# MorphIQ-Labs/VectorWave

Measured on AMD Instinct MI355X. Metric: Msamples/sec MODWT fwd+inv db4 L=6, batch 4096×4096 fp64 @ 1/2/4/8 GPU, higher is better.
Workload: dtype f64

## Files before the change

### vectorwave_amd/csrc/vw_device.h

```cpp
#pragma once
#include <hip/hip_runtime.h>
#include <cstdint>
#include <type_traits>
#include "vw_internal.h"

#pragma clang fp contract(off)

namespace vw {

template <typename T> struct VT;
template <> struct VT<double> { typedef double v __attribute__((ext_vector_type(2))); static constexpr int V = 2; };
template <> struct VT<float>  { typedef float  v __attribute__((ext_vector_type(4))); static constexpr int V = 4; };

__device__ __forceinline__ double fma_t(double a, double b, double c) { return __builtin_fma(a, b, c); }
__device__ __forceinline__ float fma_t(float a, float b, float c) { return __builtin_fmaf(a, b, c); }

template <bool FMA, typename T>
__device__ __forceinline__ T madd(T acc, T x, T f) {
  if constexpr (FMA) return fma_t(x, f, acc);
  else return acc + x * f;
}

#ifndef VW_PK_F32
#define VW_PK_F32 0
// ... 920 lines not shown
  const size_t plane = (size_t)p.B * (size_t)N;

  T reg[NV][V];
  T dnext[NV][V];
  load_row_regs<T, NV>(reg, p.approx + b * (size_t)N, N, nvec, vec_ok, p.approx_zero != 0);
  load_row_regs<T, NV>(dnext, p.details + (size_t)(p.J - 1) * plane + b * (size_t)N, N, nvec, vec_ok,
                       p.lv[p.J - 1].use_d == 0);
  wait_vmem();
  regs_to_level<T, L, NV>(A, reg, nvec, N, p.lv[p.J - 1], 0, (const T*)nullptr, p.approx_zero != 0);
  regs_to_level<T, L, NV>(D, dnext, nvec, N, p.lv[p.J - 1], 0, (const T*)nullptr, p.lv[p.J - 1].use_d == 0, p.thr,
                          thr_of(p.J), p.soft);

  for (int j = p.J; j >= 1; --j) {
    const LevelDesc lv = p.lv[j - 1];
    lds_barrier();
    if (j > 1) {
      load_row_regs<T, NV>(dnext, p.details + (size_t)(j - 2) * plane + b * (size_t)N, N, nvec, vec_ok,
                           p.lv[j - 2].use_d == 0);
    }
    for_vecs<L, NV>(nvec, [&](int k, int w) {
      T acc[V];
#pragma unroll
      for (int e = 0; e < V; ++e) acc[e] = T(0);
      inv_pair<T, L, FMA>(A, D, w * V, lv.s, lv.dir_a, p.lo, p.hi, p.taps, acc);
#pragma unroll
      for (int e = 0; e < V; ++e) {
        asm volatile("" : "+v"(acc[e]));
        reg[k][e] = acc[e];
      }
    });
    if (j == 1) {
      for_vecs<L, NV>(nvec, [&](int k, int w) { store_vec<VW_INV_STORE_AUX>(p.y + b * (size_t)N, w * V, N, vec_ok, reg[k]); });
    } else {
      const LevelDesc ln = p.lv[j - 2];
      lds_barrier();
      regs_to_level<T, L, NV>(A, reg, nvec, N, ln, 0, (const T*)nullptr);
      wait_vmem();
      regs_to_level<T, L, NV>(D, dnext, nvec, N, ln, 0, (const T*)nullptr, ln.use_d == 0, p.thr, thr_of(j - 1), p.soft);
    }
  }
}

template <typename T, int L, bool FMA, int NV, int LH = L>
__global__ void VW_FUSED_BOUNDS(NV, VW_FUSED_W((L > LH ? L : LH), 6)) k_inverse_db(const InvArgs<T> p) {
  constexpr int V = VT<T>::V;
  extern __shared__ __attribute__((aligned(16))) unsigned char smem[];
  T* const X = reinterpret_cast<T*>(smem) + p.hlpad_a;
  T* const Y = reinterpret_cast<T*>(smem) + p.region_d + p.hlpad_d;
  const long long b = p.rev ? p.B - 1 - (long long)blockIdx.x : (long long)blockIdx.x;
  const int N = p.N;
  const int nvec = (N + V - 1) / V;
  const bool vec_ok = (L > 0) || p.vec_io != 0;
  auto thr_of = [&](int j) { return p.thr ? load_uniform(p.thr + (size_t)(j - 1) * (size_t)p.thr_ld + (size_t)b) : T(0); };
  const size_t plane = (size_t)p.B * (size_t)N;

  T acc[NV][V];
  T dreg[NV][V];
  load_row_regs<T, NV>(acc, p.approx + b * (size_t)N, N, nvec, vec_ok, p.approx_zero != 0);
  load_row_regs<T, NV>(dreg, p.details + (size_t)(p.J - 1) * plane + b * (size_t)N, N, nvec, vec_ok,
                       p.lv[p.J - 1].use_d == 0);
  wait_vmem();
  regs_to_level<T, L, NV>(X, acc, nvec, N, p.lv[p.J - 1], 0, (const T*)nullptr, p.approx_zero != 0);

  for (int j = p.J; j >= 1; --j) {
    const LevelDesc lv = p.lv[j - 1];
    lds_barrier();
    wait_vmem();
    regs_to_level<T, L, NV>(Y, dreg, nvec, N, lv, 0, (const T*)nullptr, lv.use_d == 0, p.thr, thr_of(j), p.soft);
    if (j > 1)
      load_row_regs<T, NV>(dreg, p.details + (size_t)(j - 2) * plane + b * (size_t)N, N, nvec, vec_ok,
                           p.lv[j - 2].use_d == 0);
    zero_regs<T, NV>(acc);
    inv_row<T, L, FMA, NV>(X, nvec, lv.s, lv.dir_a, lv.off_a, p.lo, p.taps, p.level_ct, acc);
    lds_barrier();
    inv_row<T, LH, FMA, NV>(Y, nvec, lv.s, lv.dir_d, lv.off_d, p.hi, p.taps_hi, p.level_ct, acc);
    if (j > 1) regs_to_level<T, L, NV>(X, acc, nvec, N, p.lv[j - 2], 0, (const T*)nullptr);
  }
  for_vecs<L, NV>(nvec, [&](int k, int w) { store_vec<VW_INV_STORE_AUX>(p.y + b * (size_t)N, w * V, N, vec_ok, acc[k]); });
}

#ifndef VW_INV_W
#define VW_INV_W 6
#endif
template <typename T, int L, bool FMA, int NV, bool FULL = false, int LH = L>
__global__ void VW_FUSED_BOUNDS(NV, VW_FUSED_W((L > LH ? L : LH), VW_INV_W)) k_inverse_seq(const InvArgs<T> p) {
  constexpr int V = VT<T>::V;
  extern __shared__ __attribute__((aligned(16))) unsigned char smem[];
  T* R = reinterpret_cast<T*>(smem) + p.hlpad_a;
  const long long b = p.rev ? p.B - 1 - (long long)blockIdx.x : (long long)blockIdx.x;
  const int N = p.N;
  const int nvec = (N + V - 1) / V;
  const bool vec_ok = (L > 0) || p.vec_io != 0;
  auto thr_of = [&](int j) { return p.thr ? load_uniform(p.thr + (size_t)(j - 1) * (size_t)p.thr_ld + (size_t)b) : T(0); };
  const size_t plane = (size_t)p.B * (size_t)N;

  T acc[NV][V];
  T dreg[NV][V];
  T nf = T(0);
  const bool nfp = p.nf_flag != nullptr;
  load_row_regs<T, NV, FULL>(acc, p.approx + b * (size_t)N, N, nvec, vec_ok, p.approx_zero != 0);
  load_row_regs<T, NV, FULL>(dreg, p.details + (size_t)(p.J - 1) * plane + b * (size_t)N, N, nvec, vec_ok,
                       p.lv[p.J - 1].use_d == 0);
  wait_vmem();
  regs_to_level<T, L, NV, FULL>(R, acc, nvec, N, p.lv[p.J - 1], 0, (const T*)nullptr, p.approx_zero != 0);

  for (int j = p.J; j >= 1; --j) {
    const LevelDesc lv = p.lv[j - 1];
    lds_barrier();
    zero_regs<T, NV>(acc);
    inv_row<T, L, FMA, NV, FULL>(R, nvec, lv.s, lv.dir_a, lv.off_a, p.lo, p.taps, p.level_ct, acc);
    lds_barrier();
    wait_vmem();
    regs_to_level<T, L, NV, FULL>(R, dreg, nvec, N, lv, 0, (const T*)nullptr, lv.use_d == 0, p.thr, thr_of(j), p.soft);
    if (j > 1)
      load_row_regs<T, NV, FULL>(dreg, p.details + (size_t)(j - 2) * plane + b * (size_t)N, N, nvec, vec_ok,
                           p.lv[j - 2].use_d == 0);
    lds_barrier();
    inv_row<T, LH, FMA, NV, FULL>(R, nvec, lv.s, lv.dir_d, lv.off_d, p.hi, p.taps_hi, p.level_ct, acc);
    if (j > 1) {
      lds_barrier();
      regs_to_level<T, L, NV, FULL>(R, acc, nvec, N, p.lv[j - 2], 0, (const T*)nullptr);
    }
  }
  for_vecs<L, NV, FULL>(nvec, [&](int k, int w) { store_vec<VW_INV_STORE_AUX, FULL>(p.y + b * (size_t)N, w * V, N, vec_ok, acc[k]); });
  if (nfp) {
    nf_probe_rows<T, L, NV, V, FULL>(nf, acc, nvec);
    nf_flag_row<T>(p.nf_flag, b, nf);
  }
}

}

#include "vw_blk.h"

namespace vw {

template <typename T>
__device__ __forceinline__ T halo_value_global(const T* __restrict__ src, int idx, int N, int mode, int npow2,
                                               const T* hist_b, int hist_len) {
  if (idx >= 0 && idx < N) return src[idx];
  switch (mode) {
    case kHaloPeriodic: { int r = idx % N; if (r < 0) r += N; return src[r]; }
    case kHaloSymmetric: return src[sym_index(idx, N)];
    case kHaloFftPad: { int r = idx < 0 ? idx + npow2 : idx; return (r >= 0 && r < N) ? src[r] : T(0); }
    case kHaloHistory: return (idx < 0 && idx >= -hist_len) ? hist_b[hist_len + idx] : T(0);
    default: return T(0);
  }
}

template <typename T>
__device__ __forceinline__ void tile_to_lds(T* buf, const T* __restrict__ src, int N, int ts, int lo_q, int hi_q,
                                            int mode, int npow2, const T* hist_b, int hist_len, const T* thr,
                                            T thr_b, int soft, bool zero, bool vec_ok = false) {
  constexpr int V = VT<T>::V;
  using vec = typename VT<T>::v;
  int qa = lo_q, qb = lo_q;
  if (vec_ok && !zero) {
    qa = max(lo_q, -ts);
    qa = (qa + V - 1) / V * V;
    qb = min(hi_q, N - ts);
    qb = qb >= qa ? qa + (qb - qa) / V * V : qa;
  }
  for (int q = qa + (int)threadIdx.x * V; q < qb; q += blockDim.x * V) {
    vec v = __builtin_nontemporal_load(reinterpret_cast<const vec*>(src + ts + q));
    if (thr) {
#pragma unroll
      for (int e = 0; e < V; ++e) v[e] = threshold_t(v[e], thr_b, soft);
    }
// ... 767 lines not shown
```

### vectorwave_amd/csrc/vw_internal.h

```cpp
#pragma once
#include <hip/hip_runtime.h>
#include <atomic>
#include <cstdint>
#include "vw_taps.h"

namespace vw {

constexpr int kMaxTaps = 64;
constexpr int kMaxLevels = 24;
constexpr int kNV = 8;
constexpr int kMaxThreads = 1024;
constexpr int kLdsBytes = 160 * 1024;
constexpr int kSweepMinS = 16;
constexpr int kSweepChunk = 128;

enum HaloMode : int {
  kHaloPeriodic = 0,
  kHaloZero = 1,
  kHaloSymmetric = 2,
  kHaloFftPad = 3,
  kHaloHistory = 4
};

struct LevelDesc {
  int s;
  int hl, hr;
  int mode;
  int dir_a;
  int off_a;
  int dir_d;
  int off_d;
  int use_d;
  int hist_len;
  int own;
  int il_a, il_b;
  int ir_a, ir_b;
  int vs, ve;
};

template <typename T>
struct FwdArgs {
  const T* x;
  long long ldx;
  T* details;
  T* approx;
  long long B;
  int N;
  int J;
  int npow2;
  int hlpad;
  int region1;
  int vec_io;
  int unrolled;
  int dma_nt;
  int level_ct;
  int validate;
  int rev;
  unsigned long long* bad;
  T* hist[kMaxLevels];
  int hist_update;
  int taps;
  int taps_hi;
  int tap_lds;
  int blk_tight;
  int* nf_flag;
  T lo[kMaxTaps];
  T hi[kMaxTaps];
  LevelDesc lv[kMaxLevels];
};

template <typename T>
struct InvArgs {
  const T* details;
  const T* approx;
  T* y;
  long long B;
  int N;
  int J;
  int hlpad_a, hlpad_d;
  int region_d;
  int vec_io;
  int pair;
  int unrolled;
  int level_ct;
  int full;
  int db;
  int blk;
  int approx_zero;
  int rev;
  const T* thr;
  long long thr_ld;
  int soft;
  int taps;
  int taps_hi;
  int tap_lds;
  int blk_tight;
  int* nf_flag;
  T lo[kMaxTaps];
  T hi[kMaxTaps];
  LevelDesc lv[kMaxLevels];
};

template <typename T>
struct LevelArgs {
  const T* src_a;
  long long lda;
  const T* src_d;
  const T* src_d2;
  const T* thr2;
  int use_d2;
  const T* src_d3;
  const T* thr3;
  int use_d3;
  T* out_a;
  T* out_d;
  const T* hist;
  long long B;
  int N;
  int tile;
  int hlpad;
  int region_d, hlpad_d;
  int pair;
  const T* thr;
  int soft;
  int use_d;
  int vec_io;
  int validate;
  unsigned long long* bad;
  int npow2;
  int taps;
  T lo[kMaxTaps];
  T hi[kMaxTaps];
  LevelDesc lv;
};

constexpr int kMaxGroup = 8;
constexpr int kMultiInvNI = 8;
constexpr int kMultiPF = 6;
template <typename T>
struct MultiArgs {
  const T* src_a;
  long long lda;
  const T* src_d[kMaxGroup];
  T* out_d[kMaxGroup];
  T* out_a;
  const T* thr[kMaxGroup];
  long long B;
  int N;
  int tile;
  int nlev;
  int s0;
  int ext[kMaxGroup + 1];
  int region;
  int vec_io;
  int soft;
  int taps;
  int rblk;
  int pf;
  int pad;
  int* nf_flag;
  int slack;
  int ni;
  T lo[kMaxTaps];
  T hi[kMaxTaps];
};

enum ThrMethod { kThrUniversal = 0, kThrSure = 1, kThrMinimax = 2, kThrBayes = 3, kThrFixed = 4 };
constexpr int kSigmaRegN = 16384;
// ... 194 lines not shown
```

### vectorwave_amd/csrc/vw_inv.hip

```cpp
#include "vw_launch.h"
#include <algorithm>

namespace vw {

template <typename T, int L, bool FMA, int NV>
static hipError_t run_inverse_fused_nv(const InvArgs<T>& a, int threads, int lds, hipStream_t st) {
  static LdsOnce configured_pair, configured_seq, configured_db, configured_blk, configured_full;
  const bool blk = L > 0 && NV != 2 && a.blk && !a.pair && !a.db;
  auto k = a.pair ? k_inverse_fused<T, L, FMA, NV> : a.db ? k_inverse_db<T, L, FMA, NV> : k_inverse_seq<T, L, FMA, NV>;
  if constexpr (NV != 2) {
    if (blk) k = k_inverse_blk<T, (L > 0 ? L : 2), FMA, NV>;
  }
  bool full = false;
  if constexpr (NV == 4 && L > 0 && L <= 8) {
    full = a.full && !a.pair && !a.db && !blk;
    if (full) k = k_inverse_seq<T, L, FMA, NV, true>;
  }
  hipError_t e = set_lds(k, lds, a.pair ? &configured_pair : a.db ? &configured_db
                                 : blk ? &configured_blk : full ? &configured_full : &configured_seq);
  if (e != hipSuccess) return e;
  hipLaunchKernelGGL(k, dim3((unsigned)a.B), dim3(threads), lds, st, a);
  return hipGetLastError();
}

template <typename T, int L, bool FMA>
static hipError_t run_inverse_fused(const InvArgs<T>& a, int threads, int lds, int nv, hipStream_t st) {
  if constexpr (L > 0 && L <= 8) {
    if (nv == 2) return run_inverse_fused_nv<T, L, FMA, 2>(a, threads, lds, st);
  }
  return nv <= 4 ? run_inverse_fused_nv<T, L, FMA, 4>(a, threads, lds, st) : run_inverse_fused_nv<T, L, FMA, 8>(a, threads, lds, st);
}

template <typename T, int L, int LH, bool FMA, int NV>
static hipError_t run_inverse_bi_nv(const InvArgs<T>& a, int threads, int lds, hipStream_t st) {
  static LdsOnce configured_seq, configured_db;
  auto k = a.db ? k_inverse_db<T, L, FMA, NV, LH> : k_inverse_seq<T, L, FMA, NV, false, LH>;
  hipError_t e = set_lds(k, lds, a.db ? &configured_db : &configured_seq);
  if (e != hipSuccess) return e;
  hipLaunchKernelGGL(k, dim3((unsigned)a.B), dim3(threads), lds, st, a);
  return hipGetLastError();
}
template <typename T, int L, int LH>
static hipError_t run_inverse_bi(const InvArgs<T>& a, int threads, int lds, bool fma, int nv, hipStream_t st) {
  if (nv <= 4) return fma ? run_inverse_bi_nv<T, L, LH, true, 4>(a, threads, lds, st) : run_inverse_bi_nv<T, L, LH, false, 4>(a, threads, lds, st);
  return fma ? run_inverse_bi_nv<T, L, LH, true, 8>(a, threads, lds, st) : run_inverse_bi_nv<T, L, LH, false, 8>(a, threads, lds, st);
}

template <typename T>
hipError_t launch_inverse_fused(const InvArgs<T>& a, int threads, int lds, bool fma, int nv, hipStream_t st) {
  if (a.taps_hi != a.taps) {
    if (a.pair || a.blk || nv == 2) return hipErrorInvalidValue;
    if (a.unrolled) {
#define VW_CASE(lo, hi) if (a.taps == lo && a.taps_hi == hi) return run_inverse_bi<T, lo, hi>(a, threads, lds, fma, nv, st);
      VW_TAP_PAIR_LIST(VW_CASE)
#undef VW_CASE
    }
    return run_inverse_bi<T, 0, 0>(a, threads, lds, fma, nv, st);
  }
  switch (a.unrolled ? a.taps : 0) {
#define VW_CASE(n) \
    case n: return fma ? run_inverse_fused<T, n, true>(a, threads, lds, nv, st) : run_inverse_fused<T, n, false>(a, threads, lds, nv, st);
    VW_TAP_LIST(VW_CASE)
#undef VW_CASE
    default:
      return fma ? run_inverse_fused<T, 0, true>(a, threads, lds, nv, st) : run_inverse_fused<T, 0, false>(a, threads, lds, nv, st);
  }
}
template hipError_t launch_inverse_fused<VW_T>(const InvArgs<VW_T>&, int, int, bool, int, hipStream_t);
}
```

### vectorwave_amd/csrc/vw_plan.cpp

```cpp
#include "vw_plan.h"

#include <algorithm>
#include <cstdio>
#include <cstdlib>
#include <cstring>
#include <type_traits>

namespace vw {

struct TuningKey {
  const char* name;
  void (*set)(Tuning& t, const Tuning& d, int v);
};
#define VW_KEY(name, stmt) {name, [](Tuning& t, const Tuning& d, int v) { (void)d; stmt; }}
static const TuningKey kTuningTable[] = {
    VW_KEY("VW_NV", t.nv = v < 0 ? d.nv : v <= 4 ? 4 : 8),
    VW_KEY("VW_FWD_PERSIST", t.fwd_persist = v < 0 ? d.fwd_persist : v != 0),
    VW_KEY("VW_FWD_BUF", t.fwd_buf = v < 0 ? d.fwd_buf : v),
    VW_KEY("VW_FORCE_TILED", t.force_tiled = v > 0),
    VW_KEY("VW_FWD_REV", t.fwd_rev = v < 0 ? 0 : v),
    VW_KEY("VW_INV_REV", t.inv_rev = v < 0 ? 0 : v),
    VW_KEY("VW_FWD_TILE", t.fwd_tile = v < 0 ? 0 : v),
    VW_KEY("VW_MULTI", t.multi = v < 0 ? d.multi : v != 0),
    VW_KEY("VW_MULTI_DIV", t.multi_div = v <= 0 ? d.multi_div : v),
    VW_KEY("VW_MULTI_TILE", t.multi_tile = v < 0 ? 0 : v),
    VW_KEY("VW_INV_BUF", t.inv_buf = v < 0 ? 0 : v),
    VW_KEY("VW_INV_TILE", t.inv_tile = v < 0 ? 0 : v),
    VW_KEY("VW_MULTI_RBLK", t.multi_rblk = v < 0 ? d.multi_rblk : v),
    VW_KEY("VW_MULTI_PF", t.multi_pf = v < 0 ? d.multi_pf : v),
    VW_KEY("VW_MULTI_PAD", t.multi_pad = v < 0 ? d.multi_pad : v),
    VW_KEY("VW_MULTI_INV_TILE", t.multi_inv_tile = v < 0 ? 0 : v),
    VW_KEY("VW_NO_SWEEP", t.no_sweep = v > 0),
    VW_KEY("VW_SWEEP_QC", t.sweep_qc = v >= 16 ? v : d.sweep_qc),
    VW_KEY("VW_UNROLL_MAX", t.unroll_max = v < 0 ? d.unroll_max : v),
    VW_KEY("VW_BLK", t.blk = v < 0 ? d.blk : v),
    VW_KEY("VW_FWD_NV", t.fwd_nv = v < 0 ? d.fwd_nv : v),
    VW_KEY("VW_INV_NV", t.inv_nv = v < 0 ? d.inv_nv : v),
    VW_KEY("VW_DEEP", t.deep = v < 0 ? d.deep : v != 0; t.deep_inv = v < 0 ? d.deep_inv : v != 0),
    VW_KEY("VW_DEEP_INV", t.deep_inv = v < 0 ? d.deep_inv : v != 0),
    VW_KEY("VW_DEEP_LDS", t.deep_lds = v <= 0 ? d.deep_lds : v),
    VW_KEY("VW_DEEP_WAVES", t.deep_waves = v <= 0 ? d.deep_waves : v),
    VW_KEY("VW_DEEP_PF_FWD", t.deep_pf_fwd = v <= 0 ? d.deep_pf_fwd : std::min(v, 16)),
    VW_KEY("VW_DEEP_PF_INV", t.deep_pf_inv = v <= 0 ? d.deep_pf_inv : std::min(v, 16)),
    VW_KEY("VW_SWEEP2", t.sweep2 = v < 0 ? d.sweep2 : v),
    VW_KEY("VW_SWEEP2_KA", t.sweep2_ka = v == 16 ? 16 : v == 8 ? 8 : d.sweep2_ka),
    VW_KEY("VW_SWEEP2_UC", t.sweep2_uc = v >= 32 ? v : d.sweep2_uc),
    VW_KEY("VW_SWEEP2_R", t.sweep2_r = v == 32 ? 32 : 0),
    VW_KEY("VW_SWEEP2_MINB", t.sweep2_minb = v < 0 ? d.sweep2_minb : v),
    VW_KEY("VW_BLK_FWD8", t.blk_fwd8 = v < 0 ? d.blk_fwd8 : v),
    VW_KEY("VW_DMA_NT", t.dma_nt = v < 0 ? d.dma_nt : v),
    VW_KEY("VW_MULTI_NI", t.multi_ni = v < 0 ? d.multi_ni : v == 4 ? 4 : 8),
    VW_KEY("VW_MFMA", t.mfma = v < 0 ? d.mfma : v),
    VW_KEY("VW_REF_GRID", t.ref_grid = v < 0 ? d.ref_grid : v),
    VW_KEY("VW_LEVEL_CT", t.level_ct = v < 0 ? d.level_ct : v != 0),
    VW_KEY("VW_ENERGY_FUSED", t.energy_fused = v < 0 ? d.energy_fused : v),
    VW_KEY("VW_BI", t.bi = v < 0 ? d.bi : v & 7),
    VW_KEY("VW_BI_LISTED", t.bi_listed = v < 0 ? d.bi_listed : v != 0),
};
#undef VW_KEY

bool set_tuning(Tuning& t, const char* key, int v) {
  const Tuning d;
  for (const TuningKey& k : kTuningTable)
    if (!strcmp(k.name, key)) { k.set(t, d, v); return true; }
  return false;
}

Tuning read_tuning() {
  Tuning t;
  const Tuning d;
  for (const TuningKey& k : kTuningTable) {
    const char* e = getenv(k.name);
    if (e) k.set(t, d, *e == '\0' ? 1 : atoi(e));
  }
  return t;
}


int max_levels(int64_t N, int L) {
  if (L <= 0 || N <= L) return 0;
  int max_level = 1;
  const long long lm1 = L - 1;
  while (max_level < 10) {
    const long long scaled = lm1 * (1LL << (max_level - 1)) + 1LL;
    if (scaled > N) break;
    max_level++;
  }
  return max_level - 1;
}

int64_t upsampled_length(int L, int level) {
  const int64_t up = (level <= 1) ? 1 : ((int64_t)1 << (level - 1));
  return (int64_t)(L - 1) * up + 1;
}

int ref_mode(int boundary) {
  return boundary == VW_PERIODIC ? kHaloPeriodic : boundary == VW_ZERO_PADDING ? kHaloZero : kHaloSymmetric;
}

static void sym_decide(int wid, int L, int level, int* ap, int* dh, int* dp, int* dg) {
  int detailPlus = 1, deltaG = 0, deltaH = 0;
  const bool isHaar = L <= 2;
  int approxPlus = isHaar ? 1 : 0;
  if (isHaar) {
    deltaG = 0;
    deltaH = (level <= 1) ? 0 : -1;
  } else if (wid == VW_WID_DB6) {
    deltaH = (level <= 1) ? 0 : -1;
    deltaG = (level >= 3) ? 1 : 0;
  } else if (wid == VW_WID_DB8) {
    deltaH = (level <= 1) ? 0 : 1;
    deltaG = (level >= 2) ? 1 : 0;
  } else if (wid == VW_WID_SYM4) {
    approxPlus = 1; detailPlus = 0; deltaH = 0; deltaG = 0;
  } else if (wid == VW_WID_SYM8) {
    if (level <= 1) { deltaH = 0; deltaG = 0; }
    else if (level == 2) { deltaH = 1; deltaG = 0; }
    else { deltaH = 1; deltaG = 1; }
  } else if (wid == VW_WID_COIF2) {
    approxPlus = 1; deltaH = (level <= 1) ? 0 : 1; detailPlus = 0; deltaG = 0;
  } else if (wid == VW_WID_COIF3) {
    detailPlus = 0;
    if (level <= 1) { deltaH = 0; deltaG = 0; } else { deltaH = -1; deltaG = 1; }
  } else if (L >= 12) {
    if (level <= 1) { deltaH = 0; deltaG = 0; }
    else { const bool even = level % 2 == 0; deltaH = even ? 0 : -1; deltaG = even ? 0 : -1; }
  } else {
    if (level <= 1) { deltaH = 0; deltaG = 0; } else { deltaH = -1; deltaG = 0; }
  }
  *ap = approxPlus; *dh = deltaH; *dp = detailPlus; *dg = deltaG;
}

static int compute_tau(int base_len, int level) {
  const int lm1 = base_len - 1;
  if (level <= 1) return std::max(0, lm1 / 2);
  const long long up = 1LL << (level - 1);
  const long long Lj = (long long)lm1 * up + 1LL;
  const long long tau = (Lj - 1LL) / 2LL;
  if (tau < 0) return 0;
  if (tau > 2147483647LL) return 2147483647;
// ... 514 lines not shown
  const int tmax = (int)((c.N + V - 1) / V * V - 1);
  for (int j = 1; j <= c.J; ++j) {
    LevelDesc& d = lv[j - 1];
    memset(&d, 0, sizeof(d));
    d.s = 1 << (j - 1);
    d.use_d = (c.detail_mask >> (j - 1)) & 1u;
    d.mode = ref_mode(c.boundary);
    if (c.boundary == VW_SYMMETRIC && !c.single_level) {
      int ap, dh, dp, dg;
      sym_decide(c.wid, Llo, j, &ap, &dh, &dp, &dg);
      const int tauH = compute_tau(Llo, j) + dh;
      const int tauG = compute_tau(Lhi, j) + dg;
      d.dir_a = ap ? 1 : -1; d.off_a = ap ? -tauH : tauH;
      d.dir_d = dp ? 1 : -1; d.off_d = dp ? -tauG : tauG;
    } else if (c.boundary == VW_SYMMETRIC) {
      const int dir = (c.flags & VW_FLAG_BATCH_SYM_INVERSE) ? 1 : -1;
      d.dir_a = d.dir_d = dir; d.off_a = d.off_d = 0;
    } else {
      d.dir_a = d.dir_d = 1; d.off_a = d.off_d = 0;
    }
    int hl = 0, hr = 0;
    branch_extent((int)c.N, tmax, c.L, d.s, d.dir_a, d.off_a, &hl, &hr);
    branch_extent((int)c.N, tmax, c.L, d.s, d.dir_d, d.off_d, &hl, &hr);
    d.hl = hl; d.hr = hr;
    *max_hl = std::max(*max_hl, hl);
    *max_hr = std::max(*max_hr, hr);
  }
}

template <typename T>
static bool plan_inverse_fused(const Tuning& tu, const InvCall<T>& c, bool pair, int max_hl, int max_hr,
                               InvPlan<T>* p, bool bi = false) {
  constexpr int V = vec_width<T>();
  const int64_t N = c.N, nvec = (N + V - 1) / V;
  const int L = c.L, J = c.J;
  const bool periodic = c.boundary == VW_PERIODIC;
  InvArgs<T>& a = p->args;
  const int hlpad = (int)round_up(max_hl, V);
  const int64_t region = round_up(hlpad + nvec * V + max_hr + V, V);
  int threads = 0, lds = 0, nv = 4;
  const bool blk_pref = !bi && tu.blk > 0 && L >= tu.blk && has_unrolled_taps(L) && periodic;
  bool db = !pair && (tu.inv_buf ? tu.inv_buf == 2 : (c.B <= 2LL * c.cus && !blk_pref));
  bool fused = false, fit = false;
  const bool inv_io = (N % V == 0) && aligned16(c.details) && aligned16(c.approx) && aligned16(c.y);
  const int inv_nv2 = (tu.inv_nv == 2 && inv_io && L <= 8 && L <= tu.unroll_max && has_unrolled_taps(L)) ? 2 : 0;
  if (!tu.force_tiled) {
    if (pair || db) fused = fused_plan(tu, N, V, sizeof(T), 2 * region, &threads, &nv, &lds, &fit, inv_nv2);
    if (!fused && !pair) {
      db = false;
      fused = fused_plan(tu, N, V, sizeof(T), region, &threads, &nv, &lds, &fit, inv_nv2);
    }
  }
  if (!fused) return false;
  for (int j = 0; j < J; ++j) set_halo_images(a.lv[j], N, 0, V, threads, nv);
  a.db = db ? 1 : 0;
  a.hlpad_a = hlpad; a.hlpad_d = hlpad; a.region_d = (int)region;
  a.vec_io = inv_io;
  a.unrolled = a.vec_io && fit && L <= tu.unroll_max;
  a.pair = pair;
  a.rev = tu.inv_rev;
  a.level_ct = tu.level_ct;
  a.full = tu.level_ct && a.unrolled && (int64_t)threads * nv == nvec;
  p->kernel = pair ? kInvPair : db ? kInvDb : kInvSeq;
  if (!bi && tu.blk > 0 && L >= tu.blk && has_unrolled_taps(L) && nv != 2 && !pair && !db && periodic && a.unrolled &&
      (int64_t)threads * nv == nvec) {
    const BlkPlan b = blk_plan<T>(a.lv, J, L, nvec, nv, true);
    a.blk_tight = b.tight;
    if (b.ok) {
      a.blk = 1;
      a.tap_lds = (int)(b.buf * V);
      lds = (int)(b.buf * 16) + 2 * L * (int)sizeof(T);
      p->kernel = kInvBlk;
    }
  }
  if (std::is_same<T, float>::value) {
    bool ok = !bi && (tu.mfma & 2) && p->fma && !pair && periodic && a.vec_io;
    for (int j = 0; ok && j < J; ++j) ok = plus_zero(a.lv[j]);
    if (const int mfma_lds = mfma_layout(ok, L, J, N, 0, &a.hlpad_a, &a.tap_lds)) {
      lds = mfma_lds;
      p->kernel = kInvMfma;
    }
  }
  p->nf_probed = p->ref_nf && (p->kernel == kInvSeq || p->kernel == kInvBlk);
  p->threads = threads; p->nv = nv; p->lds = lds;
  return true;
}

template <typename T>
static void inverse_multi_layout(const Tuning& tu, const LevelDesc* lv, int j0, int g, int L, int mtile,
                                 MultiArgs<T>& m) {
  constexpr int V = vec_width<T>();
  m.region = (int)round_up(mtile + m.ext[g - 1] + V, V);
  m.rblk = tu.multi_rblk;
  m.pf = tu.multi_pf && m.vec_io && (int64_t)(mtile + m.ext[g - 1]) / V <= (int64_t)kMultiPF * 256;
  m.pad = tu.multi_pad && m.pf && m.rblk && has_unrolled_taps(L);
  if (m.pad) {
    const int nvmax = (mtile + m.ext[g - 1]) / V + 1;
    m.region = (nvmax + nvmax / 8 + 1) * V;
  }
  m.slack = 160;
  m.ni = kMultiInvNI;
  if (tu.multi_ni == 4 && sizeof(T) == 8 && m.pad) {
    auto fits = [&](int64_t t) {
      if ((t + m.ext[g - 1]) / V > (int64_t)kMultiPF * 256) return false;
      for (int k = 0; k < g; ++k) {
        const int64_t s = lv[j0 - 1 + k].s, M = s % V == 0 ? s / V : 0;
        const int64_t nv = (t + (k > 0 ? m.ext[k - 1] : 0)) / V;
        const bool blk = M == 1 || M == 2 || M == 4 || M == 8;
        if (blk ? (nv + 4 * M - 1) / (4 * M) * M > 256 : nv > 4 * 256) return false;
      }
      return true;
    };
    int64_t t = mtile;
    while (t >= 512 && !fits(t)) t -= 64 * V;
    if (t >= 512) {
      m.ni = 4;
      m.tile = (int)t;
      const int nvmax = (int)((t + m.ext[g - 1]) / V) + 1;
      m.region = (nvmax + nvmax / 4 + 1) * V;
    }
  }
}

template <typename T>
static void plan_inverse_levels(const Tuning& tu, const InvCall<T>& c, bool pair, InvPlan<T>* p) {
  constexpr int V = vec_width<T>();
  const int64_t N = c.N;
  const int L = c.L, J = c.J;
  const bool periodic = c.boundary == VW_PERIODIC;
  const LevelDesc* lv = p->args.lv;
  const int tile_max = tu.inv_tile ? tu.inv_tile / V * V : 1024;
  const size_t plane = (size_t)c.B * (size_t)N;
  p->res.ws_bytes = 2 * plane * sizeof(T) + 256;
  const StepAlign al{c.approx, c.y, c.details, plane * sizeof(T)};
  auto plane_al = [&](int j) { return !lv[j - 1].use_d || al.plane(j - 1); };
  const int mtile = tu.multi_inv_tile >= 64 * V ? tu.multi_inv_tile / V * V : multi_tile<T>(tu);
  int groups[kMaxLevels], start_of[kMaxLevels + 1] = {};
  level_groups(tu, lv, J, L, V, mtile, !pair && periodic, groups);
  for (int j = 1; j <= J; ++j) {
    if (groups[j - 1] < 2) continue;
    int64_t ext = 0;
    for (int k = 0; k < groups[j - 1]; ++k) ext += round_up((int64_t)(L - 1) * lv[j - 1 + k].s, V);
    if ((mtile + ext) / V <= (int64_t)kMultiInvNI * 256) start_of[j + groups[j - 1] - 1] = j;
  }
  char in_group[kMaxLevels + 1] = {};
  for (int e = 1; e <= J; ++e)
    for (int k = start_of[e]; start_of[e] > 0 && k <= e; ++k) in_group[k] = 1;
  int cur = c.approx_zero ? kBufNone : kBufIn;
  for (int j = J; j >= 1; --j) {
    const int nxt = cur == kBufWs0 ? kBufWs1 : kBufWs0;
    if (!pair && periodic && !in_group[j] && al.buf(cur) && aligned16(c.details) && aligned16(c.y) &&
        deep_plan<T>(tu, lv, j, j, L, N, true, nullptr)) {
      int jl = j;
      while (jl > 1 && !in_group[jl - 1] && deep_plan<T>(tu, lv, jl - 1, j, L, N, true, nullptr)) --jl;
      PlanStep<T>& s = add_step(p->steps, kStepDeep, jl, j, cur, jl == 1 ? kBufOut : nxt);
      s.lds = deep_plan<T>(tu, lv, jl, j, L, N, true, &s.deep);
      deep_segments<T>(tu, c.cus, c.B, &s.deep);
      s.deep.lda = N; s.deep.B = c.B; s.deep.taps = L; s.deep.soft = c.soft;
      cur = s.dst;
      j = jl;
      continue;
    }
    if (start_of[j] > 0) {
      const int j0 = start_of[j], g = j - j0 + 1;
      PlanStep<T>& s = add_step(p->steps, kStepMulti, j0, j, cur, j0 == 1 ? kBufOut : nxt);
      MultiArgs<T>& m = s.multi;
      s.probe = p->ref_nf && j0 == 1;
      bool io = al.buf(cur) && al.buf(s.dst);
      for (int k = 0; k < g; ++k) {
        io = io && plane_al(j0 + k);
        m.ext[k] = (k > 0 ? m.ext[k - 1] : 0) + (int)round_up((int64_t)(L - 1) * lv[j0 - 1 + k].s, V);
      }
      m.B = c.B; m.N = (int)N; m.tile = mtile; m.nlev = g; m.s0 = lv[j0 - 1].s;
      m.vec_io = (N % V == 0) && io;
      m.soft = c.soft; m.taps = L;
      inverse_multi_layout<T>(tu, lv, j0, g, L, mtile, m);
      s.lds = (int)((2 * m.region + m.slack * V) * sizeof(T));
      cur = s.dst;
      j = j0;
      continue;
    }
    if (tu.sweep2 && !tu.deep_inv && !tu.no_sweep && !pair && j >= 2 && has_unrolled_taps(L)) {
      int G = 0, ka = 0, R = 0;
      for (int levels = std::min(tu.sweep2 >= 3 ? 3 : 2, j); levels >= 2 && !G; --levels)
        if (sweepg_plan<T>(tu, lv, j, levels, L, N, in_group, start_of, &ka, &R)) G = levels;
      if (G) {
        PlanStep<T>& s = add_step(p->steps, kStepSweepG, j - G + 1, j, cur, j == G ? kBufOut : nxt);
        LevelArgs<T>& a = s.lvl;
        a.lv = lv[j - 1];
        a.use_d = lv[j - 1].use_d;
        a.use_d2 = lv[j - 2].use_d;
        if (G == 3) a.use_d3 = lv[j - 3].use_d;
        a.soft = c.soft;
        a.B = c.B; a.N = (int)N; a.taps = L;
        s.G = G == 2 ? 2 : 4; s.ka = ka; s.R = R;
        a.tile = (int)round_up(tu.sweep2_uc, s.G * ka);
        cur = s.dst;
        j -= G - 1;
        continue;
      }
    }
    const bool sweep = lv[j - 1].s >= kSweepMinS && has_unrolled_taps(L) && !tu.no_sweep;
    PlanStep<T>& s = add_step(p->steps, sweep ? kStepSweep : kStepTile, j, j, cur, j == 1 ? kBufOut : nxt);
    LevelArgs<T>& a = s.lvl;
    a.lv = lv[j - 1];
    const int hp = (int)round_up(a.lv.hl, V);
    const int64_t fit = ((int64_t)kLdsBytes / (int64_t)sizeof(T) / 2 - hp - a.lv.hr - 2 * V) / V * V;
    const int tile = (int)std::min<int64_t>(tile_max, fit);
    if (tile < 64 * V) return plan_error(p, VW_ERR_UNSUPPORTED, "level %d halo exceeds LDS", j);
    const int64_t reg = round_up(hp + tile + a.lv.hr + V, V);
    a.use_d = a.lv.use_d;
    a.B = c.B; a.N = (int)N; a.tile = sweep ? tu.sweep_qc : tile; a.hlpad = hp; a.hlpad_d = hp; a.region_d = (int)reg;
    a.pair = pair; a.soft = c.soft; a.taps = L;
    a.vec_io = (N % V == 0) && al.buf(s.dst) && al.buf(cur) && plane_al(j);
    s.lds = sweep ? 0 : (int)(2 * reg * sizeof(T));
    cur = s.dst;
  }
  p->nf_probed = !p->steps.empty() && p->steps.back().probe;
}

template <typename T>
static void plan_inverse_taps(const Tuning& tu, const InvCall<T>& call, int taps, InvPlan<T>* p, bool bi = false) {
  InvCall<T> c = call;
  const int Llo = call.L, Lhi = hi_taps(call);
  const bool pair = c.single_level || c.boundary == VW_ZERO_PADDING;
  if (pair && Lhi < Llo)
    return plan_error(p, VW_ERR_UNSUPPORTED, "pairwise inverse: the reference indexes past its high-pass array (%d < %d taps)",
                      Lhi, Llo);
  c.L = pair ? Llo : taps;
  c.Lhi = 0;
  p->fma = c.flags & VW_FLAG_FMA;
  const bool padded = !pair && (c.L != Llo || c.L != Lhi);
  p->ref_nf = (c.flags & VW_FLAG_REF_NONFINITE) && (padded || (!c.single_level && c.J >= 2));
  InvArgs<T>& a = p->args;
  a.B = c.B; a.N = (int)c.N; a.J = c.J;
  a.approx_zero = c.approx_zero; a.thr_ld = c.thr_ld; a.soft = c.soft; a.taps = c.L; a.taps_hi = c.L;
  int max_hl = 0, max_hr = 0;
  inverse_levels(c, Llo, Lhi, a.lv, &max_hl, &max_hr);
  p->fused = plan_inverse_fused(tu, c, pair, max_hl, max_hr, p, bi);
  if (bi && p->fused && !pair && p->nv != 2 && (p->kernel == kInvSeq || p->kernel == kInvDb) &&
      ((tu.bi & 4) || (a.unrolled && has_unrolled_pair(Llo, Lhi)))) {
    a.taps = Llo; a.taps_hi = Lhi;
    a.unrolled = a.unrolled && has_unrolled_pair(Llo, Lhi);
    a.full = 0;
  }
  if (!p->fused) plan_inverse_levels(tu, c, pair, p);
  reserve_ref<T>(tu, c.cus, c.B, c.N, p);
}

template <typename T>
void plan_forward(const Tuning& tu, const FwdCall<T>& c, FwdPlan<T>* p) {
  const int Lmax = std::max(c.L, hi_taps(c)), taps = listed_taps(tu, Lmax, c.L != hi_taps(c));
  if ((tu.bi & 1) && c.L != hi_taps(c) && !c.hist) {
    plan_forward_taps(tu, c, Lmax, p, true);
    if (p->error != VW_OK || p->args.taps_hi != p->args.taps) return;
    *p = FwdPlan<T>();
  }
  plan_forward_taps(tu, c, taps, p);
  if (p->error != VW_OK && taps != Lmax) {
    *p = FwdPlan<T>();
    plan_forward_taps(tu, c, Lmax, p);
  }
}

template <typename T>
void plan_inverse(const Tuning& tu, const InvCall<T>& c, InvPlan<T>* p) {
  const int Lmax = std::max(c.L, hi_taps(c)), taps = listed_taps(tu, Lmax, c.L != hi_taps(c));
  if ((tu.bi & 2) && c.L != hi_taps(c)) {
    plan_inverse_taps(tu, c, Lmax, p, true);
    if (p->error == VW_OK && p->args.taps_hi != p->args.taps) return;
    *p = InvPlan<T>();
  }
  plan_inverse_taps(tu, c, taps, p);
  if (p->error != VW_OK && taps != Lmax) {
    *p = InvPlan<T>();
    plan_inverse_taps(tu, c, Lmax, p);
  }
}

template void plan_forward<float>(const Tuning&, const FwdCall<float>&, FwdPlan<float>*);
template void plan_forward<double>(const Tuning&, const FwdCall<double>&, FwdPlan<double>*);
template void plan_inverse<float>(const Tuning&, const InvCall<float>&, InvPlan<float>*);
template void plan_inverse<double>(const Tuning&, const InvCall<double>&, InvPlan<double>*);

}
```

### vectorwave_amd/csrc/vw_plan.h

```cpp
#pragma once
#include "../../include/vectorwave_amd.h"
#include "vw_internal.h"
#include "vw_deep.h"

#include <vector>

namespace vw {

struct Tuning {
  int nv = 4;
  bool fwd_persist = true;
  int fwd_buf = 0;
  bool force_tiled = false;
  int fwd_rev = 0, inv_rev = 0;
  int dma_nt = -1;
  int fwd_tile = 0;
  bool multi = true;
  int multi_div = 4;
  int multi_tile = 0;
  int inv_buf = 0;
  int inv_tile = 0;
  int multi_rblk = 1;
  int multi_pf = 1;
  int multi_pad = 1;
  int multi_inv_tile = 0;
  int multi_ni = 4;
  bool no_sweep = false;
  int sweep_qc = kSweepChunk;
  int unroll_max = kMaxTaps;
  int blk = 10;
  bool deep = true;
  bool deep_inv = false;
  int deep_lds = 80;
  int deep_waves = 4;
  int deep_pf_fwd = 1;
  int deep_pf_inv = 1;
  int fwd_nv = 0;
  int inv_nv = 0;
  int sweep2 = 3;
  int sweep2_ka = 8;
  int sweep2_uc = 2048;
  int sweep2_r = 0;
  int sweep2_minb = 64;
  int blk_fwd8 = 1;
  int ref_grid = 0;
  int level_ct = 1;
  int mfma = 0;
  int energy_fused = 1;
  int bi = 3;
  int bi_listed = 1;
};

bool set_tuning(Tuning& t, const char* key, int v);
Tuning read_tuning();

int max_levels(int64_t N, int L);
int64_t upsampled_length(int L, int level);
int ref_mode(int boundary);

template <typename T>
struct FwdCall {
  const T* x = nullptr;
  int64_t B = 0, N = 0, ldx = 0;
  const double* lo = nullptr;
  const double* hi = nullptr;
  int L = 0, boundary = VW_PERIODIC, J = 1;
  unsigned flags = 0;
  T* details = nullptr;
  T* approx = nullptr;
  bool single_level = false;
  int mode_override = -1;
  T* const* hist = nullptr;
  bool hist_update = false;
  T* const* hist_snap = nullptr;
  bool hist_first = false;
  int cus = 256;
  int Lhi = 0;
};

template <typename T>
struct InvCall {
  const T* details = nullptr;
  const T* approx = nullptr;
  int64_t B = 0, N = 0;
  const double* lo = nullptr;
  const double* hi = nullptr;
  int L = 0, wid = VW_WID_OTHER, boundary = VW_PERIODIC, J = 1;
  unsigned detail_mask = ~0u;
  int approx_zero = 0;
  unsigned flags = 0;
  T* y = nullptr;
  bool single_level = false;
  const T* thr = nullptr;
  int soft = 0;
  int64_t thr_ld = 0;
  int cus = 256;
  int Lhi = 0;
};

enum PlanKernel : int {
  kFwdFused, kFwdPersist, kFwdBlk, kFwdMfma,
  kInvPair, kInvSeq, kInvDb, kInvBlk, kInvMfma,
  kStepDeep, kStepMulti, kStepSweepG, kStepSweep, kStepTile
};
enum PlanBuf : int { kBufNone, kBufIn, kBufWs0, kBufWs1, kBufOut };

template <typename T>
struct PlanStep {
  int kind;
  int jlo, jhi;
  int src, dst;
  int lds;
  int G, ka, R;
  int probe;
  int hist_update;
  union {
    LevelArgs<T> lvl;
    MultiArgs<T> multi;
    DeepArgs<T> deep;
  };
};

struct PlanReserve {
  size_t ws_bytes = 0;
  int64_t nf_rows = 0;
  int ref_grid = 0;
};

template <typename T, typename Args>
struct Plan {
  int error = VW_OK;
  char msg[96] = "";
// ... 28 lines not shown
```

Measured before the change: 46340.

## Add a plain full-slab fp64 inverse MODWT kernel path for short periodic filters

Adds a specialised inverse-sequence kernel for fp64, NV=4, short unrolled filters on periodic boundaries with no thresholding. It replaces general row loads and stores with raw buffer loads and stores at fixed slab offsets, writes the halo to LDS directly, and uses sched barriers to keep register pressure and scheduling under control. It also adds a waves-per-EU launch-bound option (6 or 8) through a tuning key. The aim is to cut address arithmetic, predication and register use in the hot inverse loop. The cost is an extra kernel variant whose eligibility depends on plan-time checks.

```diff
diff --git a/vectorwave_amd/csrc/vw_device.h b/vectorwave_amd/csrc/vw_device.h
--- a/vectorwave_amd/csrc/vw_device.h
+++ b/vectorwave_amd/csrc/vw_device.h
@@ -1026,8 +1026,152 @@
 #ifndef VW_INV_W
 #define VW_INV_W 6
 #endif
-template <typename T, int L, bool FMA, int NV, bool FULL = false, int LH = L>
-__global__ void VW_FUSED_BOUNDS(NV, VW_FUSED_W((L > LH ? L : LH), VW_INV_W)) k_inverse_seq(const InvArgs<T> p) {
+template <int NV, typename F>
+__device__ __forceinline__ void plain_vecs(unsigned slab, F&& fn) {
+#pragma unroll
+  for (int k = 0; k < NV; ++k) {
+    unsigned vb = threadIdx.x * 16u;
+    asm volatile("" : "+v"(vb));
+    fn(k, vb + k * slab);
+    __builtin_amdgcn_sched_barrier(0);
+  }
+}
+
+template <typename T, int NV>
+__device__ __forceinline__ void plain_load_row(T (&r)[NV][VT<T>::V], const T* row, unsigned slab) {
+  using vec = typename VT<T>::v;
+  const __amdgpu_buffer_rsrc_t rs = row_rsrc(row);
+  unsigned vb = threadIdx.x * 16u;
+  asm volatile("" : "+v"(vb));
+#pragma unroll
+  for (int k = 0; k < NV; ++k) {
+    const vec v = __builtin_bit_cast(vec, __builtin_amdgcn_raw_buffer_load_b128(rs, vb, k * slab, 2));
+#pragma unroll
+    for (int e = 0; e < VT<T>::V; ++e) r[k][e] = v[e];
+  }
+}
+template <typename T, int NV>
+__device__ __forceinline__ void plain_store_row(T* row, const T (&r)[NV][VT<T>::V], unsigned slab) {
+  using vec = typename VT<T>::v;
+  const __amdgpu_buffer_rsrc_t rs = row_rsrc(row);
+  unsigned vb = threadIdx.x * 16u;
+  asm volatile("" : "+v"(vb));
+#pragma unroll
+  for (int k = 0; k < NV; ++k) {
+    vec o;
+#pragma unroll
+    for (int e = 0; e < VT<T>::V; ++e) o[e] = r[k][e];
+    __builtin_amdgcn_raw_buffer_store_b128(__builtin_bit_cast(vw_i4, o), rs, vb, k * slab, 2);
+  }
+}
+
+template <typename T, int NV>
+__device__ __forceinline__ void plain_to_level(T* R, const T (&r)[NV][VT<T>::V], unsigned slab, int N, int hr, int own) {
+  constexpr int V = VT<T>::V;
+  using vec = typename VT<T>::v;
+  plain_vecs<NV>(slab, [&](int k, unsigned vb) {
+    vec o;
+#pragma unroll
+    for (int e = 0; e < V; ++e) o[e] = r[k][e];
+    T* const at = reinterpret_cast<T*>(reinterpret_cast<unsigned char*>(R) + vb);
+    *reinterpret_cast<vec*>(at) = o;
+    if (k == 0 && own && vb < (unsigned)hr * (unsigned)sizeof(T)) {
+#pragma unroll
+      for (int e = 0; e < V; ++e)
+        if (vb + e * (unsigned)sizeof(T) < (unsigned)hr * (unsigned)sizeof(T)) at[N + e] = o[e];
+    }
+  });
+  if (!own) {
+    lds_barrier();
+    for (int q = threadIdx.x; q < hr; q += blockDim.x) R[N + q] = R[q];
+  }
+}
+
+template <typename T, int L, bool FMA, int NV, int RIF, int S>
+__device__ __forceinline__ void plain_row_s(const T* R, unsigned slab, int s, const T* f, T (&acc)[NV][VT<T>::V]) {
+  constexpr int V = VT<T>::V;
+  using vec = typename VT<T>::v;
+  plain_vecs<NV>(slab, [&](int k, unsigned vb) {
+    const T* const at = reinterpret_cast<const T*>(reinterpret_cast<const unsigned char*>(R) + vb);
+    if constexpr (S < 0) {
+      inv_window<T, L, FMA, -S, 1>(at, 0, f, acc[k]);
+    } else {
+      const unsigned a0 = lds_base(at);
+#pragma unroll
+      for (int i = 0; i < L; ++i) {
+        const vec v = S > 0 ? lds_vec_at<vec>(a0 + (unsigned)(i * S * (int)sizeof(T)))
+                            : *reinterpret_cast<const vec*>(at + i * s);
+        vmadd<FMA>(acc[k], v, f[i]);
+        if (i % RIF == RIF - 1) __builtin_amdgcn_sched_barrier(0);
+      }
+    }
+#pragma unroll
+    for (int e = 0; e < V; ++e) asm volatile("" : "+v"(acc[k][e]));
+  });
+}
+template <typename T, int L, bool FMA, int NV, int RIF>
+__device__ __forceinline__ void plain_row(const T* R, unsigned slab, int s, const T* f, T (&acc)[NV][VT<T>::V]) {
+  constexpr int V = VT<T>::V;
+  if (s == 1) return plain_row_s<T, L, FMA, NV, RIF, -1>(R, slab, s, f, acc);
+  if constexpr (V == 4) {
+    if (s == 2) return plain_row_s<T, L, FMA, NV, RIF, -2>(R, slab, s, f, acc);
+  }
+  switch (s) {
+#define VW_CASE(n)                                                                             \
+    case n:                                                                                    \
+      if constexpr (n % V == 0) return plain_row_s<T, L, FMA, NV, RIF, n>(R, slab, s, f, acc); \
+      break;
+    VW_CT_SPACINGS(VW_CASE)
+#undef VW_CASE
+    default: break;
+  }
+  plain_row_s<T, L, FMA, NV, RIF, 0>(R, slab, s, f, acc);
+}
+
+template <typename T, int L, bool FMA, int NV, int W>
+__device__ __forceinline__ void inverse_seq_plain(const InvArgs<T>& p) {
+  constexpr int V = VT<T>::V;
+  constexpr int RIF = W >= 8 ? 3 : 4;
+  extern __shared__ __attribute__((aligned(16))) unsigned char smem[];
+  T* const R = reinterpret_cast<T*>(smem) + p.hlpad_a;
+  const size_t N = (size_t)p.N;
+  const size_t row = (size_t)blockIdx.x * N, plane = (size_t)p.B * N;
+  const unsigned slab = blockDim.x * 16u;
+
+  T acc[NV][V];
+  T dreg[NV][V];
+  plain_load_row<T, NV>(acc, p.approx + row, slab);
+  plain_load_row<T, NV>(dreg, p.details + (size_t)(p.J - 1) * plane + row, slab);
+  wait_vmem();
+  plain_to_level<T, NV>(R, acc, slab, p.N, p.lv[p.J - 1].hr, p.lv[p.J - 1].own);
+
+  for (int j = p.J; j >= 1; --j) {
+    const int s = p.lv[j - 1].s;
+    lds_barrier();
+    zero_regs<T, NV>(acc);
+    plain_row<T, L, FMA, NV, RIF>(R, slab, s, p.lo, acc);
+    lds_barrier();
+    wait_vmem();
+    plain_to_level<T, NV>(R, dreg, slab, p.N, p.lv[j - 1].hr, p.lv[j - 1].own);
+    if (j > 1)
+      plain_load_row<T, NV>(dreg, p.details + (size_t)(j - 2) * plane + row, slab);
+    lds_barrier();
+    plain_row<T, L, FMA, NV, RIF>(R, slab, s, p.hi, acc);
+    if (j > 1) {
+      lds_barrier();
+      plain_to_level<T, NV>(R, acc, slab, p.N, p.lv[j - 2].hr, p.lv[j - 2].own);
+    }
+  }
+  plain_store_row<T, NV>(p.y + row, acc, slab);
+}
+
+template <typename T, int L, bool FMA, int NV, bool FULL = false, int LH = L, int W = VW_INV_W, bool PLAIN = false>
+__global__ void VW_FUSED_BOUNDS(NV, VW_FUSED_W((L > LH ? L : LH), W)) k_inverse_seq(const InvArgs<T> p) {
+  if constexpr (PLAIN) {
+    static_assert(FULL && L > 0 && L <= 8 && LH == L && NV == 4, "the plain form is a full-slab form of the short filters");
+    inverse_seq_plain<T, L, FMA, NV, W>(p);
+    return;
+  }
   constexpr int V = VT<T>::V;
   extern __shared__ __attribute__((aligned(16))) unsigned char smem[];
   T* R = reinterpret_cast<T*>(smem) + p.hlpad_a;
diff --git a/vectorwave_amd/csrc/vw_internal.h b/vectorwave_amd/csrc/vw_internal.h
--- a/vectorwave_amd/csrc/vw_internal.h
+++ b/vectorwave_amd/csrc/vw_internal.h
@@ -84,6 +84,8 @@
   int unrolled;
   int level_ct;
   int full;
+  int plain;
+  int waves;
   int db;
   int blk;
   int approx_zero;
diff --git a/vectorwave_amd/csrc/vw_inv.hip b/vectorwave_amd/csrc/vw_inv.hip
--- a/vectorwave_amd/csrc/vw_inv.hip
+++ b/vectorwave_amd/csrc/vw_inv.hip
@@ -5,7 +5,7 @@
 
 template <typename T, int L, bool FMA, int NV>
 static hipError_t run_inverse_fused_nv(const InvArgs<T>& a, int threads, int lds, hipStream_t st) {
-  static LdsOnce configured_pair, configured_seq, configured_db, configured_blk, configured_full;
+  static LdsOnce configured_pair, configured_seq, configured_db, configured_blk, configured_full, configured_plain[2];
   const bool blk = L > 0 && NV != 2 && a.blk && !a.pair && !a.db;
   auto k = a.pair ? k_inverse_fused<T, L, FMA, NV> : a.db ? k_inverse_db<T, L, FMA, NV> : k_inverse_seq<T, L, FMA, NV>;
   if constexpr (NV != 2) {
@@ -16,8 +16,16 @@
     full = a.full && !a.pair && !a.db && !blk;
     if (full) k = k_inverse_seq<T, L, FMA, NV, true>;
   }
+  LdsOnce* plain = nullptr;
+  if constexpr (NV == 4 && L > 0 && L <= 8 && std::is_same<T, double>::value) {
+    if (full && a.plain && !a.thr && !a.nf_flag && !a.approx_zero && !a.rev) {
+      const bool w8 = a.waves == 8;
+      k = w8 ? k_inverse_seq<T, L, FMA, NV, true, L, 8, true> : k_inverse_seq<T, L, FMA, NV, true, L, 6, true>;
+      plain = &configured_plain[w8];
+    }
+  }
   hipError_t e = set_lds(k, lds, a.pair ? &configured_pair : a.db ? &configured_db
-                                 : blk ? &configured_blk : full ? &configured_full : &configured_seq);
+                                 : blk ? &configured_blk : plain ? plain : full ? &configured_full : &configured_seq);
   if (e != hipSuccess) return e;
   hipLaunchKernelGGL(k, dim3((unsigned)a.B), dim3(threads), lds, st, a);
   return hipGetLastError();
diff --git a/vectorwave_amd/csrc/vw_plan.cpp b/vectorwave_amd/csrc/vw_plan.cpp
--- a/vectorwave_amd/csrc/vw_plan.cpp
+++ b/vectorwave_amd/csrc/vw_plan.cpp
@@ -56,6 +56,7 @@
     VW_KEY("VW_ENERGY_FUSED", t.energy_fused = v < 0 ? d.energy_fused : v),
     VW_KEY("VW_BI", t.bi = v < 0 ? d.bi : v & 7),
     VW_KEY("VW_BI_LISTED", t.bi_listed = v < 0 ? d.bi_listed : v != 0),
+    VW_KEY("VW_INV_WAVES", t.inv_waves = v == 6 || v == 8 ? v : d.inv_waves),
 };
 #undef VW_KEY
 
@@ -736,6 +737,12 @@
     }
   }
   p->nf_probed = p->ref_nf && (p->kernel == kInvSeq || p->kernel == kInvBlk);
+  bool plain = a.full && p->kernel == kInvSeq && sizeof(T) == 8 && nv == 4 && L <= 8 && periodic && !c.thr &&
+               !c.approx_zero && !a.rev && !p->ref_nf;
+  for (int j = 0; plain && j < J; ++j)
+    plain = a.lv[j].use_d && plus_zero(a.lv[j]) && a.lv[j].hl == 0 && a.lv[j].hr <= N;
+  a.plain = plain ? 1 : 0;
+  a.waves = tu.inv_waves;
   p->threads = threads; p->nv = nv; p->lds = lds;
   return true;
 }
@@ -897,6 +904,7 @@
     a.taps = Llo; a.taps_hi = Lhi;
     a.unrolled = a.unrolled && has_unrolled_pair(Llo, Lhi);
     a.full = 0;
+    a.plain = 0;
   }
   if (!p->fused) plan_inverse_levels(tu, c, pair, p);
   reserve_ref<T>(tu, c.cus, c.B, c.N, p);
diff --git a/vectorwave_amd/csrc/vw_plan.h b/vectorwave_amd/csrc/vw_plan.h
--- a/vectorwave_amd/csrc/vw_plan.h
+++ b/vectorwave_amd/csrc/vw_plan.h
@@ -48,6 +48,7 @@
   int mfma = 0;
   int energy_fused = 1;
   int bi = 3;
+  int inv_waves = 6;
   int bi_listed = 1;
 };
 
```

Result: faster. 47110 (median of 6 runs) (+1.7%).
